# craftsangjae/instance-segmentation-road-project

Hardware: AMD Instinct MI355X
Metric: images/sec at 1024x1024 (MaskLab inference hot path, full forward) (higher is better)
Workload: dtype f32; 1 GPU; resnext50_full_b8_1024; per_gpu_batch=8, global_batch=8, height=1024, width=1024, parallelism=dp1, hipgraph=False, inputs=resident in HBM, weights=random init (cls logits x8 so NMS / mask head run at full load)

## Files before the change

instance-segmentation-road-project_amd/csrc/conv_wino.hip:

```cpp
#include "common.h"

namespace {

constexpr int WMAXP = ML_CONV_MAX_PROBLEMS;
constexpr int WT = 64;
constexpr int WN = 32;
constexpr int WK = 8;
constexpr int PT_LD = 132;
constexpr int WB_LD = 516;
constexpr int WCHUNK = WK * WN * 16;

struct WProblem {
    ml_conv2d_desc d;
    int TH, TW, T;
    int MB, NB, nchunks;
};

struct WArgs {
    int n;
    int start[WMAXP + 1];
    WProblem p[WMAXP];
};

__device__ __forceinline__ void bt_d_b(const float d[16], float v[16]) {
    float t[16];
#pragma unroll
    for (int j = 0; j < 4; ++j) {
        t[0 * 4 + j] = d[0 * 4 + j] - d[2 * 4 + j];
        t[1 * 4 + j] = d[1 * 4 + j] + d[2 * 4 + j];
        t[2 * 4 + j] = d[2 * 4 + j] - d[1 * 4 + j];
        t[3 * 4 + j] = d[1 * 4 + j] - d[3 * 4 + j];
    }
#pragma unroll
    for (int i = 0; i < 4; ++i) {
        v[i * 4 + 0] = t[i * 4 + 0] - t[i * 4 + 2];
        v[i * 4 + 1] = t[i * 4 + 1] + t[i * 4 + 2];
        v[i * 4 + 2] = t[i * 4 + 2] - t[i * 4 + 1];
        v[i * 4 + 3] = t[i * 4 + 1] - t[i * 4 + 3];
    }
}

__global__ void __launch_bounds__(256, 2) conv_wino_kernel(const WArgs args) {
    __shared__ __attribute__((aligned(16))) float lds_p[WT * PT_LD];
    __shared__ __attribute__((aligned(16))) float lds_w[WK * WB_LD];
    __shared__ double lds_gn[4][4];

    int pi = 0;
    while (pi + 1 < args.n && (int)blockIdx.x >= args.start[pi + 1]) ++pi;
    const WProblem &P = args.p[pi];
    const ml_conv2d_desc &p = P.d;
    const int b = (int)blockIdx.x - args.start[pi];
    const int g = b / (8 * P.NB), rr = b - g * 8 * P.NB;
    const int nt = rr >> 3;
    const int mt = g * 8 + (rr & 7);
    if (mt >= P.MB) return;
    if (p.live) {
        const int lv = max(1, *p.live), tpi0 = P.TH * P.TW;
        const int b0 = mt * WT / tpi0, b1 = min(mt * WT + WT, P.T) - 1;
        bool any = false;
        for (int bi = b0; bi <= b1 / tpi0 && !any; ++bi) any = bi % p.live_period < lv;
        if (!any) return;
    }

    const int tid = threadIdx.x, lane = tid & 63, wave = tid >> 6;
    const int r = lane & 15, kq = lane >> 4;
    const int tpi = P.TH * P.TW;

    int pix[8];
#pragma unroll
    for (int i = 0; i < 8; ++i) {
        const int idx = tid + 256 * i;
        const int tile = idx >> 5, px = (idx >> 1) & 15;
        const int gt = mt * WT + tile;
        pix[i] = -1;
        if (gt < P.T) {
            const int bi = gt / tpi, rem = gt - bi * tpi;
            const int ty = rem / P.TW, tx = rem - ty * P.TW;
            const int y = 2 * ty - 1 + (px >> 2), x = 2 * tx - 1 + (px & 3);
            if (y >= 0 && y < p.H && x >= 0 && x < p.W) pix[i] = (bi * p.H + y) * p.W + x;
        }
    }
    const size_t cstride = (size_t)p.in_cstride;
    const float *in = p.in + p.in_coff + ((tid & 1) << 2);
    const float *wsrc = p.wgt + (size_t)nt * P.nchunks * WCHUNK + tid * 4;

    f32x4 rp[8], rw[4];
    auto load_chunk = [&](int c) {
#pragma unroll
        for (int i = 0; i < 8; ++i) {
            rp[i] = f32x4{0.f, 0.f, 0.f, 0.f};
            if (pix[i] >= 0) rp[i] = *reinterpret_cast<const f32x4 *>(in + (size_t)pix[i] * cstride + c * WK);
        }
#pragma unroll
        for (int i = 0; i < 4; ++i) rw[i] = *reinterpret_cast<const f32x4 *>(wsrc + (size_t)c * WCHUNK + i * 1024);
    };

    f32x4 acc[2][16];
#pragma unroll
    for (int t = 0; t < 2; ++t)
#pragma unroll
        for (int q = 0; q < 16; ++q) acc[t][q] = f32x4{0.f, 0.f, 0.f, 0.f};

    load_chunk(0);
    for (int c = 0; c < P.nchunks; ++c) {
        __syncthreads();
#pragma unroll
        for (int i = 0; i < 8; ++i) {
            const int idx = tid + 256 * i;
            *reinterpret_cast<f32x4 *>(lds_p + (idx >> 5) * PT_LD + (idx & 31) * 4) = rp[i];
        }
#pragma unroll
        for (int i = 0; i < 4; ++i) {
            const int idx = tid + 256 * i;
            *reinterpret_cast<f32x4 *>(lds_w + (idx >> 7) * WB_LD + (idx & 127) * 4) = rw[i];
        }
        __syncthreads();
        if (c + 1 < P.nchunks) load_chunk(c + 1);
#pragma unroll
        for (int s = 0; s < 2; ++s) {
            const int ch = 4 * s + kq;
            const float *pa = lds_p + (wave * 16 + r) * PT_LD + ch;
            float d[16], v[16];
#pragma unroll
            for (int px = 0; px < 16; ++px) d[px] = pa[px * WK];
            bt_d_b(d, v);
#pragma unroll
            for (int t = 0; t < 2; ++t) {
                const float *pb = lds_w + ch * WB_LD + (16 * t + r) * 16;
#pragma unroll
                for (int pq = 0; pq < 4; ++pq) {
                    const f32x4 bq = *reinterpret_cast<const f32x4 *>(pb + 4 * pq);
#pragma unroll
                    for (int e = 0; e < 4; ++e)
                        acc[t][4 * pq + e] = __builtin_amdgcn_mfma_f32_16x16x4f32(v[4 * pq + e], bq[e], acc[t][4 * pq + e], 0, 0, 0);
                }
            }
        }
    }

    const bool gn = p.gn_partials != nullptr;
    double gs[2] = {0.0, 0.0}, gq[2] = {0.0, 0.0};
    long long f0 = 0;
    if (gn) {
        const int gt0 = mt * WT;
        const int bi = gt0 / tpi, rem = gt0 - bi * tpi, ty = rem / P.TW, tx = rem - ty * P.TW;
        f0 = ((long long)(bi * p.Ho + 2 * ty) * p.Wo + 2 * tx) >> 7;
    }
    const float lo = 0.f, hi = (p.act == ML_ACT_RELU6) ? 6.f : 3.402823466e38f;
    const bool clampv = p.act == ML_ACT_RELU || p.act == ML_ACT_RELU6;
#pragma unroll
    for (int i = 0; i < 4; ++i) {
        const int gt = mt * WT + wave * 16 + kq * 4 + i;
        if (gt >= P.T) continue;
        const int bi = gt / tpi, rem = gt - bi * tpi;
        const int ty = rem / P.TW, tx = rem - ty * P.TW;
        const int oy = 2 * ty, ox = 2 * tx;
        const bool y1 = oy + 1 < p.Ho, x1 = ox + 1 < p.Wo;
        const size_t img = p.out_bstride ? (size_t)bi * (size_t)p.out_bstride : (size_t)bi * p.Ho * p.Wo * p.out_cstride;
        const size_t pix0 = (size_t)oy * p.Wo + ox;
#pragma unroll
        for (int t = 0; t < 2; ++t) {
            const int n = nt * WN + 16 * t + r;
            if (n >= p.cout) continue;
            float m[16];
#pragma unroll
            for (int q = 0; q < 16; ++q) m[q] = acc[t][q][i];
            float u[8];
#pragma unroll
            for (int j = 0; j < 4; ++j) {
                u[j] = m[0 * 4 + j] + m[1 * 4 + j] + m[2 * 4 + j];
                u[4 + j] = m[1 * 4 + j] - m[2 * 4 + j] - m[3 * 4 + j];
            }
            float yv[4];
#pragma unroll
            for (int a = 0; a < 2; ++a) {
                yv[2 * a] = u[4 * a + 0] + u[4 * a + 1] + u[4 * a + 2];
                yv[2 * a + 1] = u[4 * a + 1] - u[4 * a + 2] - u[4 * a + 3];
            }
            const float bv = p.bias ? p.bias[n] : 0.f;
            float *o = p.out + img + p.out_coff + n;
#pragma unroll
            for (int a = 0; a < 2; ++a)
#pragma unroll
                for (int c2 = 0; c2 < 2; ++c2) {
                    if ((a && !y1) || (c2 && !x1)) continue;
                    float val = yv[2 * a + c2] + bv;
                    if (clampv) val = __builtin_amdgcn_fmed3f(val, lo, hi);
                    else if (p.act != ML_ACT_NONE) val = ml_apply_act(val, p.act);
                    o[(pix0 + (size_t)a * p.Wo + c2) * p.out_cstride] = val;
                    if (gn) {
                        const long long m_flat = ((long long)(bi * p.Ho + oy + a) * p.Wo + ox + c2);
                        const int f = (m_flat >> 7) != f0;
                        gs[f] += (double)val;
                        gq[f] += (double)val * (double)val;
                    }
                }
        }
    }
    if (gn) {
#pragma unroll
        for (int o = 32; o > 0; o >>= 1) {
#pragma unroll
            for (int f = 0; f < 2; ++f) {
                gs[f] += __shfl_down(gs[f], o, 64);
                gq[f] += __shfl_down(gq[f], o, 64);
            }
        }
        if (lane == 0) {
            lds_gn[wave][0] = gs[0]; lds_gn[wave][1] = gq[0];
            lds_gn[wave][2] = gs[1]; lds_gn[wave][3] = gq[1];
        }
        __syncthreads();
        if (tid < 2) {
            const int gt1 = mt * WT + WT - 1;
            const int bi = gt1 / tpi, rem = gt1 - bi * tpi, ty = rem / P.TW, tx = rem - ty * P.TW;
            const long long f1 = ((long long)(bi * p.Ho + 2 * ty + 1) * p.Wo + 2 * tx + 1) >> 7;
            const long long ft = tid ? f1 : f0;
            double s = 0.0, q = 0.0;
            for (int w = 0; w < 4; ++w) { s += lds_gn[w][2 * tid]; q += lds_gn[w][2 * tid + 1]; }
            p.gn_partials[2 * (ft * 4 + nt)] = s;
            p.gn_partials[2 * (ft * 4 + nt) + 1] = q;
        }
    }
}

}

extern "C" int ml_conv2d_wino_eligible(const ml_conv2d_desc *d) {
    if (!d) return 0;
    return d->math == ML_MATH_F32 && d->KH == 3 && d->KW == 3 && d->stride == 1 && d->dil == 1 && d->pad_t == 1 &&
           d->pad_l == 1 && d->Ho == d->H && d->Wo == d->W && d->cpp_shift == 30 && d->group_cin_step == 0 &&
           !d->shuffle2x2 && !d->residual && !d->out_f16 && d->span % 32 == 0 && d->span_pad == d->span &&
           d->cout <= 128 && d->n_pad == 128;
}

int ml_conv2d_wino_gn_ok(const ml_conv2d_desc &d) {
    if (d.Ho % 2 || d.Wo % 2 || d.cout != 128 || d.out_bstride || d.act == ML_ACT_SIGMOID) return 0;
    const long long TH = d.Ho / 2, TW = d.Wo / 2;
    return (64 % TW == 0 || TW % 64 == 0) && (TH * TW) % 64 == 0;
}

int ml_conv2d_wino_launch(const ml_conv2d_desc *descs, int n, hipStream_t s) {
    ML_REQUIRE(n >= 1 && n <= WMAXP, "conv2d (winograd): need 1..%d problems", WMAXP);
    WArgs args;
    args.n = n;
    long long start = 0;
    for (int i = 0; i < n; ++i) {
        const ml_conv2d_desc &d = descs[i];
        ML_REQUIRE(ml_conv2d_wino_eligible(&d),
                   "conv2d: tile = 6 (Winograd F(2x2,3x3)) needs ML_MATH_F32, a 3x3 stride-1 undilated 'same' conv, no "
                   "groups / shuffle / residual / half output, span %% 32 == 0 and n_pad == 128");
        ML_REQUIRE(((d.in_cstride | d.in_coff) & 3) == 0 && ml_aligned16(d.in) && ml_aligned16(d.wgt),
                   "conv2d (winograd): 16-byte aligned input channels and weights");
        if (d.gn_partials)
            ML_REQUIRE(ml_conv2d_wino_gn_ok(d) && !d.live, "conv2d (winograd): gn_partials needs even Ho / Wo, Wo / 2 dividing or a "
                                                "multiple of 64, (Ho / 2) (Wo / 2) %% 64 == 0, cout = 128, dense output");
        WProblem &P = args.p[i];
        P.d = d;
        P.TH = (d.Ho + 1) / 2;
        P.TW = (d.Wo + 1) / 2;
        const long long T = (long long)d.B * P.TH * P.TW;
        ML_REQUIRE(T < (1ll << 30), "conv2d (winograd): too many tiles");
        P.T = (int)T;
        P.MB = (int)((T + WT - 1) / WT);
        P.NB = d.n_pad / WN;
        P.nchunks = d.span_pad / WK;
        args.start[i] = (int)start;
        start += (long long)(P.MB + 7) / 8 * 8 * P.NB;
        ML_REQUIRE(start < (1ll << 31), "conv2d (winograd): grid too large");
    }
    args.start[n] = (int)start;
    long long tiles128 = 0;
    bool any_gn = false;
    for (int i = 0; i < n; ++i) {
        tiles128 += ((long long)descs[i].B * descs[i].Ho * descs[i].Wo + 127) / 128 * (descs[i].n_pad / 128);
        any_gn = any_gn || descs[i].gn_partials != nullptr;
    }
    ML_REQUIRE(!any_gn || tiles128 >= ml_conv2d_gn_min_launch_tiles(),
               "conv2d (winograd): gn_partials needs a launch of ml_conv2d_gn_min_launch_tiles() tiles of 128 x 128");
    hipLaunchKernelGGL(conv_wino_kernel, dim3((unsigned)start), dim3(256), 0, s, args);
    ML_CHECK_LAUNCH("conv2d (winograd)");
    return ML_OK;
}
```

Measured before the change: 400.0 images/sec.

## Pipeline Winograd conv with buffer-to-LDS DMA, 4-slot ring and 512-thread blocks

Rewrites the Winograd F(2x2,3x3) conv main loop so input and weight chunks go straight from global memory into LDS via buffer_load_lds DMA. A four-slot ring buffer replaces the old register-staged, double-synchronised copy. Each block now has 8 waves covering 64 output channels (two 32-channel halves), and the next step's LDS operands are read while MFMAs run under explicit waitcnt and sched barriers. The aim is to hide global latency and drop the register round trip and one barrier per chunk. The cost is larger dynamic LDS, one block per CU, and a new size limit on the input span.

```diff
diff --git a/instance-segmentation-road-project_amd/csrc/conv_wino.hip b/instance-segmentation-road-project_amd/csrc/conv_wino.hip
--- a/instance-segmentation-road-project_amd/csrc/conv_wino.hip
+++ b/instance-segmentation-road-project_amd/csrc/conv_wino.hip
@@ -4,11 +4,16 @@
 
 constexpr int WMAXP = ML_CONV_MAX_PROBLEMS;
 constexpr int WT = 64;
-constexpr int WN = 32;
+constexpr int WN = 64;
 constexpr int WK = 8;
-constexpr int PT_LD = 132;
-constexpr int WB_LD = 516;
-constexpr int WCHUNK = WK * WN * 16;
+constexpr int WCHUNK = WK * 32 * 16;
+constexpr int WSTEP = 4 * 32 * 16;
+constexpr int NSLOT = 4;
+constexpr int SLOT_P = WT * 16 * 4;
+constexpr int SLOT = SLOT_P + 2 * WSTEP;
+constexpr int LDS_BYTES = NSLOT * SLOT * 4 + 8 * 4 * 8;
+constexpr unsigned OOB = 0x80000000u;
+constexpr long long SPAN_MAX = 0x7fffff00ll;
 
 struct WProblem {
     ml_conv2d_desc d;
@@ -22,6 +27,12 @@
     WProblem p[WMAXP];
 };
 
+__device__ __forceinline__ void dma16(__amdgpu_buffer_rsrc_t rsrc, float *dst, int voff) {
+#if defined(__HIP_DEVICE_COMPILE__)
+    __builtin_amdgcn_raw_ptr_buffer_load_lds(rsrc, (__attribute__((address_space(3))) void *)dst, 16, voff, 0, 0, 0);
+#endif
+}
+
 __device__ __forceinline__ void bt_d_b(const float d[16], float v[16]) {
     float t[16];
 #pragma unroll
@@ -40,10 +51,8 @@
     }
 }
 
-__global__ void __launch_bounds__(256, 2) conv_wino_kernel(const WArgs args) {
-    __shared__ __attribute__((aligned(16))) float lds_p[WT * PT_LD];
-    __shared__ __attribute__((aligned(16))) float lds_w[WK * WB_LD];
-    __shared__ double lds_gn[4][4];
+__global__ void __launch_bounds__(512, 1) conv_wino_kernel(const WArgs args) {
+    extern __shared__ __align__(16) float lds[];
 
     int pi = 0;
     while (pi + 1 < args.n && (int)blockIdx.x >= args.start[pi + 1]) ++pi;
@@ -51,7 +60,7 @@
     const ml_conv2d_desc &p = P.d;
     const int b = (int)blockIdx.x - args.start[pi];
     const int g = b / (8 * P.NB), rr = b - g * 8 * P.NB;
-    const int nt = rr >> 3;
+    const int nt2 = rr >> 3;
     const int mt = g * 8 + (rr & 7);
     if (mt >= P.MB) return;
     if (p.live) {
@@ -62,37 +71,56 @@
         if (!any) return;
     }
 
-    const int tid = threadIdx.x, lane = tid & 63, wave = tid >> 6;
+    const int tid = threadIdx.x, lane = tid & 63;
+    const int wave = __builtin_amdgcn_readfirstlane(tid >> 6);
+    const int tg = wave & 3, h = wave >> 2;
     const int r = lane & 15, kq = lane >> 4;
     const int tpi = P.TH * P.TW;
 
-    int pix[8];
-#pragma unroll
-    for (int i = 0; i < 8; ++i) {
-        const int idx = tid + 256 * i;
-        const int tile = idx >> 5, px = (idx >> 1) & 15;
-        const int gt = mt * WT + tile;
-        pix[i] = -1;
+    const int gt0 = mt * WT;
+    long long base_pix;
+    {
+        const int bi = gt0 / tpi, rem = gt0 - bi * tpi, ty = rem / P.TW;
+        base_pix = ((long long)bi * p.H + max(2 * ty - 1, 0)) * p.W;
+    }
+    const size_t cstride = (size_t)p.in_cstride;
+    const float *pin = p.in + p.in_coff + (size_t)base_pix * cstride;
+    int voff_p[2];
+    {
+        const int gt = gt0 + (wave >> 1) * 16 + r;
+        int bi = 0, ty = 0, tx = 0;
         if (gt < P.T) {
-            const int bi = gt / tpi, rem = gt - bi * tpi;
-            const int ty = rem / P.TW, tx = rem - ty * P.TW;
+            bi = gt / tpi;
+            const int rem = gt - bi * tpi;
+            ty = rem / P.TW;
+            tx = rem - ty * P.TW;
+        }
+#pragma unroll
+        for (int i = 0; i < 2; ++i) {
+            const int px = 8 * (wave & 1) + 4 * i + kq;
             const int y = 2 * ty - 1 + (px >> 2), x = 2 * tx - 1 + (px & 3);
-            if (y >= 0 && y < p.H && x >= 0 && x < p.W) pix[i] = (bi * p.H + y) * p.W + x;
-        }
-    }
-    const size_t cstride = (size_t)p.in_cstride;
-    const float *in = p.in + p.in_coff + ((tid & 1) << 2);
-    const float *wsrc = p.wgt + (size_t)nt * P.nchunks * WCHUNK + tid * 4;
-
-    f32x4 rp[8], rw[4];
-    auto load_chunk = [&](int c) {
-#pragma unroll
-        for (int i = 0; i < 8; ++i) {
-            rp[i] = f32x4{0.f, 0.f, 0.f, 0.f};
-            if (pix[i] >= 0) rp[i] = *reinterpret_cast<const f32x4 *>(in + (size_t)pix[i] * cstride + c * WK);
-        }
-#pragma unroll
-        for (int i = 0; i < 4; ++i) rw[i] = *reinterpret_cast<const f32x4 *>(wsrc + (size_t)c * WCHUNK + i * 1024);
+            voff_p[i] = (int)OOB;
+            if (gt < P.T && y >= 0 && y < p.H && x >= 0 && x < p.W)
+                voff_p[i] = (int)((((long long)bi * p.H + y) * p.W + x - base_pix) * (long long)cstride * 4);
+        }
+    }
+    const int voff_w = ((wave & 3) * 512 + r * 16 + kq * 4) * 4;
+    const float *wsrc = p.wgt + (size_t)(2 * nt2 + (wave >> 2)) * P.nchunks * WCHUNK;
+    float *dst_p = lds + (wave >> 1) * 1024 + (wave & 1) * 512;
+    float *dst_w = lds + SLOT_P + (wave >> 2) * WSTEP + (wave & 3) * 512;
+    const int nsteps = 2 * P.nchunks;
+
+    auto stage = [&](int c) __attribute__((always_inline)) {
+        const bool real = c < nsteps;
+        const __amdgpu_buffer_rsrc_t rp =
+            __builtin_amdgcn_make_buffer_rsrc((void *)(pin + c * 4), 0, real ? (int)OOB : 0, 0x00020000);
+        const __amdgpu_buffer_rsrc_t rw =
+            __builtin_amdgcn_make_buffer_rsrc((void *)(wsrc + (size_t)c * WSTEP), 0, real ? WSTEP * 4 : 0, 0x00020000);
+        const int so = (c & 3) * SLOT;
+        dma16(rp, dst_p + so, voff_p[0]);
+        dma16(rp, dst_p + so + 256, voff_p[1]);
+        dma16(rw, dst_w + so, voff_w);
+        dma16(rw, dst_w + so + 256, voff_w + 1024);
     };
 
     f32x4 acc[2][16];
@@ -101,48 +129,63 @@
 #pragma unroll
         for (int q = 0; q < 16; ++q) acc[t][q] = f32x4{0.f, 0.f, 0.f, 0.f};
 
-    load_chunk(0);
-    for (int c = 0; c < P.nchunks; ++c) {
-        __syncthreads();
-#pragma unroll
-        for (int i = 0; i < 8; ++i) {
-            const int idx = tid + 256 * i;
-            *reinterpret_cast<f32x4 *>(lds_p + (idx >> 5) * PT_LD + (idx & 31) * 4) = rp[i];
-        }
-#pragma unroll
-        for (int i = 0; i < 4; ++i) {
-            const int idx = tid + 256 * i;
-            *reinterpret_cast<f32x4 *>(lds_w + (idx >> 7) * WB_LD + (idx & 127) * 4) = rw[i];
-        }
-        __syncthreads();
-        if (c + 1 < P.nchunks) load_chunk(c + 1);
-#pragma unroll
-        for (int s = 0; s < 2; ++s) {
-            const int ch = 4 * s + kq;
-            const float *pa = lds_p + (wave * 16 + r) * PT_LD + ch;
-            float d[16], v[16];
-#pragma unroll
-            for (int px = 0; px < 16; ++px) d[px] = pa[px * WK];
-            bt_d_b(d, v);
-#pragma unroll
-            for (int t = 0; t < 2; ++t) {
-                const float *pb = lds_w + ch * WB_LD + (16 * t + r) * 16;
-#pragma unroll
-                for (int pq = 0; pq < 4; ++pq) {
-                    const f32x4 bq = *reinterpret_cast<const f32x4 *>(pb + 4 * pq);
-#pragma unroll
-                    for (int e = 0; e < 4; ++e)
-                        acc[t][4 * pq + e] = __builtin_amdgcn_mfma_f32_16x16x4f32(v[4 * pq + e], bq[e], acc[t][4 * pq + e], 0, 0, 0);
+    const float *pa_lane = lds + tg * 1024 + r * 4 + kq;
+    const float *pb_lane = lds + SLOT_P + h * WSTEP + kq * 512 + r * 4;
+    struct Ops {
+        float d[16];
+        f32x4 b[2][4];
+    };
+    auto read_ops = [&](int c, Ops &o) __attribute__((always_inline)) {
+        const float *pb = pb_lane + (c & 3) * SLOT;
+#pragma unroll
+        for (int t = 0; t < 2; ++t)
+#pragma unroll
+            for (int pq = 0; pq < 4; ++pq) o.b[t][pq] = *reinterpret_cast<const f32x4 *>(pb + t * 256 + pq * 64);
+        const float *pa = pa_lane + (c & 3) * SLOT;
+#pragma unroll
+        for (int px = 0; px < 16; ++px) o.d[px] = pa[px * 64];
+    };
+    auto step = [&](int c, const Ops &cur, Ops &nxt) __attribute__((always_inline)) {
+        asm volatile("s_waitcnt vmcnt(4) lgkmcnt(0)" ::: "memory");
+        __builtin_amdgcn_s_barrier();
+        stage(c + 3);
+        float v[16];
+        bt_d_b(cur.d, v);
+#pragma unroll
+        for (int t = 0; t < 2; ++t)
+#pragma unroll
+            for (int pq = 0; pq < 4; ++pq) {
+#pragma unroll
+                for (int e = 0; e < 4; ++e)
+                    acc[t][4 * pq + e] =
+                        __builtin_amdgcn_mfma_f32_16x16x4f32(v[4 * pq + e], cur.b[t][pq][e], acc[t][4 * pq + e], 0, 0, 0);
+                if (t == 0 && pq == 0) {
+                    __builtin_amdgcn_sched_barrier(0);
+                    read_ops(c + 1, nxt);
+                    __builtin_amdgcn_sched_barrier(0);
                 }
             }
-        }
-    }
-
+        __builtin_amdgcn_sched_barrier(0);
+    };
+
+    Ops oa, ob;
+    stage(0);
+    stage(1);
+    stage(2);
+    asm volatile("s_waitcnt vmcnt(8)" ::: "memory");
+    __builtin_amdgcn_s_barrier();
+    read_ops(0, oa);
+    for (int c = 0; c < nsteps; c += 2) {
+        step(c, oa, ob);
+        step(c + 1, ob, oa);
+    }
+    asm volatile("s_waitcnt vmcnt(0)" ::: "memory");
+
+    const int nt = 2 * nt2 + h;
     const bool gn = p.gn_partials != nullptr;
     double gs[2] = {0.0, 0.0}, gq[2] = {0.0, 0.0};
     long long f0 = 0;
     if (gn) {
-        const int gt0 = mt * WT;
         const int bi = gt0 / tpi, rem = gt0 - bi * tpi, ty = rem / P.TW, tx = rem - ty * P.TW;
         f0 = ((long long)(bi * p.Ho + 2 * ty) * p.Wo + 2 * tx) >> 7;
     }
@@ -150,7 +193,7 @@
     const bool clampv = p.act == ML_ACT_RELU || p.act == ML_ACT_RELU6;
 #pragma unroll
     for (int i = 0; i < 4; ++i) {
-        const int gt = mt * WT + wave * 16 + kq * 4 + i;
+        const int gt = gt0 + tg * 16 + kq * 4 + i;
         if (gt >= P.T) continue;
         const int bi = gt / tpi, rem = gt - bi * tpi;
         const int ty = rem / P.TW, tx = rem - ty * P.TW;
@@ -160,7 +203,7 @@
         const size_t pix0 = (size_t)oy * p.Wo + ox;
 #pragma unroll
         for (int t = 0; t < 2; ++t) {
-            const int n = nt * WN + 16 * t + r;
+            const int n = nt * 32 + 16 * t + r;
             if (n >= p.cout) continue;
             float m[16];
 #pragma unroll
@@ -198,6 +241,7 @@
         }
     }
     if (gn) {
+        double *lds_gn = reinterpret_cast<double *>(lds + NSLOT * SLOT);
 #pragma unroll
         for (int o = 32; o > 0; o >>= 1) {
 #pragma unroll
@@ -207,19 +251,21 @@
             }
         }
         if (lane == 0) {
-            lds_gn[wave][0] = gs[0]; lds_gn[wave][1] = gq[0];
-            lds_gn[wave][2] = gs[1]; lds_gn[wave][3] = gq[1];
+            lds_gn[wave * 4 + 0] = gs[0]; lds_gn[wave * 4 + 1] = gq[0];
+            lds_gn[wave * 4 + 2] = gs[1]; lds_gn[wave * 4 + 3] = gq[1];
         }
         __syncthreads();
-        if (tid < 2) {
-            const int gt1 = mt * WT + WT - 1;
+        if (tid < 4) {
+            const int hh = tid >> 1, ff = tid & 1;
+            const int gt1 = gt0 + WT - 1;
             const int bi = gt1 / tpi, rem = gt1 - bi * tpi, ty = rem / P.TW, tx = rem - ty * P.TW;
             const long long f1 = ((long long)(bi * p.Ho + 2 * ty + 1) * p.Wo + 2 * tx + 1) >> 7;
-            const long long ft = tid ? f1 : f0;
+            const long long ft = ff ? f1 : f0;
+            const int slot = 2 * nt2 + hh;
             double s = 0.0, q = 0.0;
-            for (int w = 0; w < 4; ++w) { s += lds_gn[w][2 * tid]; q += lds_gn[w][2 * tid + 1]; }
-            p.gn_partials[2 * (ft * 4 + nt)] = s;
-            p.gn_partials[2 * (ft * 4 + nt) + 1] = q;
+            for (int w = 0; w < 4; ++w) { s += lds_gn[(hh * 4 + w) * 4 + 2 * ff]; q += lds_gn[(hh * 4 + w) * 4 + 2 * ff + 1]; }
+            p.gn_partials[2 * (ft * 4 + slot)] = s;
+            p.gn_partials[2 * (ft * 4 + slot) + 1] = q;
         }
     }
 }
@@ -265,6 +311,8 @@
         P.MB = (int)((T + WT - 1) / WT);
         P.NB = d.n_pad / WN;
         P.nchunks = d.span_pad / WK;
+        const long long span = (2ll * (WT / P.TW + 2) + 2) * d.W * d.in_cstride * 4;
+        ML_REQUIRE(span <= SPAN_MAX, "conv2d (winograd): a block's input rows exceed 2 GiB (W x in_cstride too large)");
         args.start[i] = (int)start;
         start += (long long)(P.MB + 7) / 8 * 8 * P.NB;
         ML_REQUIRE(start < (1ll << 31), "conv2d (winograd): grid too large");
@@ -278,7 +326,10 @@
     }
     ML_REQUIRE(!any_gn || tiles128 >= ml_conv2d_gn_min_launch_tiles(),
                "conv2d (winograd): gn_partials needs a launch of ml_conv2d_gn_min_launch_tiles() tiles of 128 x 128");
-    hipLaunchKernelGGL(conv_wino_kernel, dim3((unsigned)start), dim3(256), 0, s, args);
+    static std::atomic<unsigned long long> lds_ok{0};
+    if (int rc = ml_ensure_dynamic_lds(reinterpret_cast<const void *>(conv_wino_kernel), LDS_BYTES, lds_ok, "conv2d (winograd)"))
+        return rc;
+    hipLaunchKernelGGL(conv_wino_kernel, dim3((unsigned)start), dim3(512), LDS_BYTES, s, args);
     ML_CHECK_LAUNCH("conv2d (winograd)");
     return ML_OK;
 }
```

Result: faster. 410.7 images/sec (median of 6 runs) (+2.7%).
